# vvvvvw/Sentinel

Measured on AMD Instinct MI355X. Metric: decided entries/sec (whole node) at 1M resources; % of HBM roofline, higher is better.
Workload: dtype int64/f64

## Files before the change

sentinel_amd/csrc/decide.hip:

```cpp
#include <hip/hip_runtime.h>
#include <stdlib.h>
#include <stdint.h>

#include "authority.h"
#include "chain.h"
#include "aux.h"
#include "pmap.h"

using namespace sg;

#define WAVE 64
#define MAXR 16
#define JMAX_FLOW 4
#define JMAX_DEG 4
#define JMAX_RL 2

__device__ __forceinline__ uint32_t lane_id() { return __lane_id(); }
__device__ __forceinline__ uint64_t lanemask_lt() {
    uint32_t l = lane_id();
    return l == 0 ? 0ull : (~0ull >> (64 - l));
}

#define J8_MAX (1u << 23)
#define SEG_ITEMS 16
// ... 89 lines not shown
    if ((threadIdx.x & 63) == 63 && tot) base = atomicAdd(ctr, tot);
    base = __shfl(base, 63, 64);
    return base + x - k;
}
__global__ __launch_bounds__(256) void k_seg_bin(Seg* __restrict__ segs, const uint32_t* __restrict__ mp, uint64_t n,
                                                 const Prog* __restrict__ prog, const uint32_t* __restrict__ prio,
                                                 uint32_t lane_max, uint32_t j1_max,
                                                 uint32_t j4_max, uint32_t force_lane, uint32_t* __restrict__ blkcnt,
                                                 uint32_t nblk, uint32_t pq_ok, uint32_t pq_wide, uint32_t* __restrict__ aux,
                                                 uint32_t* __restrict__ ashort, uint64_t* __restrict__ along,
                                                 uint64_t* __restrict__ amulti, uint32_t* __restrict__ mixc,
                                                 uint32_t* __restrict__ mix, uint32_t mix_cap,
                                                 uint32_t* __restrict__ mixlen, uint32_t mix_wide, uint32_t head_min,
                                                 const uint16_t* __restrict__ hot_tab, uint32_t nhot,
                                                 const uint32_t* __restrict__ nhotseg, uint32_t* __restrict__ need_hot,
                                                 uint32_t* __restrict__ need_blk) {
    __shared__ uint32_t cnt[N_BINS];
    for (uint32_t b = threadIdx.x; b < N_BINS; b += blockDim.x) cnt[b] = 0;
    __syncthreads();
    const uint32_t m = *mp;
    const bool pq = pq_ok && !force_lane;
    const uint32_t s = blockIdx.x * blockDim.x + threadIdx.x;
    bool aux_short = false;
    uint32_t aux_np = 0;
    uint32_t mixk = 0;
    Seg sg;
    if (s < m) {
        sg = segs[s];
        const uint32_t end = (s + 1 < m) ? segs[s + 1].start : (uint32_t)n;
        sg.len = end - sg.start;
        const Prog p = prog[sg.res];
// ... 18 lines not shown
        else if (coop) bin = (sg.len > j4_max && (p.pflags & PF_J16))
                                 ? (((p.pflags & PF_FROZEN) && sg.len <= J8_MAX) ? BIN_J8 : BIN_J16)
                                 : sg.len > j1_max ? BIN_J4 : BIN_J1;
        else {
            int lb = 31 - __clz(sg.len | 1);
            if (lb > (int)LANE_BINS - 1) lb = LANE_BINS - 1;
            const bool lite = (p.n_param == 0 || ((p.xf & XF_PLITE) && !(pm & PM_ARGL))) && !p.multi && !lane_only &&
                              (p.pflags & PF_J16) && !(p.pflags & (PF_WARM | PF_SERIAL));
            bin = (lite ? BIN_LITE : (nr <= 4 && !inline_aux) ? BIN_LANE : BIN_LANE16) + (LANE_BINS - 1 - lb);
        }
        const bool auxp = aux && (pm & PM_AUX) && !(bin >= BIN_LANE16 && bin < BIN_LANE16 + LANE_BINS);
        if (auxp) {
            if (sg.len <= AUX_SHORT) aux_short = true;
            else aux_np = (sg.len + AUX_PIECE - 1) / AUX_PIECE;
        }
        const uint32_t rank = atomicAdd(&cnt[bin], 1u);
        sg.bin = bin | (auxp ? SEG_AUXP : 0u) | (rank << 8);
        segs[s] = sg;
        if (need_blk && (bin == BIN_J4 || bin == BIN_J8 || bin == BIN_J16) && sg.len) {
            if (s < *nhotseg) {
                const uint32_t hid = hot_tab[sg.res];
                if (hid < nhot) need_hot[hid] = 1u;
            } else {
                const uint32_t b0 = sg.start >> 10, b1 = (sg.start + sg.len - 1) >> 10;
                for (uint32_t wd = b0 >> 5; wd <= (b1 >> 5); ++wd) {
                    uint32_t m32 = 0xFFFFFFFFu;
                    if (wd == (b0 >> 5)) m32 &= 0xFFFFFFFFu << (b0 & 31);
                    if (wd == (b1 >> 5)) m32 &= 0xFFFFFFFFu >> (31 - (b1 & 31));
                    atomicOr(&need_blk[wd], m32);
                }
            }
        }
    }
    if (aux) {
        const uint32_t o = wave_alloc(aux + 0, aux_short ? 1u : 0u);
        if (aux_short) ashort[o] = s;
        const uint32_t q = wave_alloc(aux + 1, aux_np);
        const uint32_t j = wave_alloc(aux + 3, aux_np ? 1u : 0u);
        if (aux_np) along[j] = ((uint64_t)s << 32) | q;
        const uint32_t u = wave_alloc(aux + 2, aux_np > 1 ? 1u : 0u);
        if (aux_np > 1) amulti[u] = ((uint64_t)s << 32) | q;
    }
    if (mix) {
        const uint32_t a = wave_alloc(mixc + 0, mixk == 1 ? 1u : 0u);
        if (mixk == 1) mix[a] = s;
        const uint32_t b = wave_alloc(mixc + 1, mixk == 2 ? 1u : 0u);
        if (mixk == 2) mix[mix_cap + b] = s;
    }
    __syncthreads();
    for (uint32_t b = threadIdx.x; b < N_BINS; b += blockDim.x) blkcnt[(uint64_t)b * nblk + blockIdx.x] = cnt[b];
}
__global__ __launch_bounds__(256) void k_seg_order(Seg* __restrict__ segs, const uint32_t* __restrict__ mp,
                                                   const uint32_t* __restrict__ off, uint32_t nblk,
                                                   uint32_t* __restrict__ order) {
    const uint32_t s = blockIdx.x * blockDim.x + threadIdx.x;
    if (s >= *mp) return;
    const uint32_t v = segs[s].bin, bin = v & 0x7F;
    order[off[(uint64_t)bin * nblk + blockIdx.x] + (v >> 8)] = s;
    segs[s].bin = v & 0xFF;
}
__global__ void k_bin_offsets(const uint32_t* __restrict__ off, uint32_t nblk, const uint32_t* __restrict__ mp,
                              uint32_t* __restrict__ out) {
    const uint32_t b = threadIdx.x;
    if (b < N_BINS) out[b] = off[(uint64_t)b * nblk];
    if (b == N_BINS) out[b] = *mp;
}

__global__ __launch_bounds__(256) void k_scatter_rec(const SEv* __restrict__ rec_o, uint64_t n,
                                                     const uint32_t* __restrict__ pos_of, SEv* __restrict__ recs,
                                                     uint32_t* __restrict__ prev, uint32_t* __restrict__ nprev,
                                                     Link* __restrict__ link, uint32_t* __restrict__ bst, uint32_t epoch,
                                                     uint32_t* __restrict__ bflags) {
    const uint64_t i = (uint64_t)blockIdx.x * blockDim.x + threadIdx.x;
    if (i >= n) return;
// ... 1541 lines not shown
#define PROF_MARK(k)                                          \
    if (prof0) {                                              \
        unsigned long long _n = __builtin_amdgcn_s_memtime(); \
        tph[k] += _n - tmA;                                   \
        tmA = _n;                                             \
    }
#else
#define PROF_MARK(k)
#endif

    uint32_t tbase = 0;
    const uint32_t lp0 = tid * EP;
    SEv nxt[EP];
    JEv ev[EP];
    uint32_t gg[EP];
    const bool skip_on = SKIP && S.skip_ok && (pg.pflags & PF_FROZEN);
    auto in_span = [&](uint32_t rel) -> bool {
        if (!SKIP) return false;
        const uint32_t ns = sh.nsp;
        for (uint32_t i = 0; i < ns; ++i)
            if (rel >= sh.spn[i].x && rel < sh.spn[i].y) return true;
        return false;
    };
    auto decode = [&](const SEv& r, uint32_t pos) -> JEv {
        JEv x;
        const bool valid = pos < sg.len;
        x.dt = valid ? r.dt : 0;
        x.cz = (uint32_t)r.cnt | ((uint32_t)r.rt << 16);
        x.kf = valid ? ((uint32_t)r.kind | JK_VALID) : 0xFFu;
        if (valid && r.kind == SG_EV_ENTRY && (r.flags & RF_PBLK)) x.kf |= JK_PB;
        x.wi = 0;
// ... 1845 lines not shown
    hipLaunchKernelGGL(k_seg_emit, dim3(nt), dim3(256), 0, st, keys, n, pos, segs, lo, sbase);
    hipLaunchKernelGGL(k_add2, dim3(1), dim3(64), 0, st, nseg, sbase, ccount);
    return hipGetLastError();
}
hipError_t launch_block_sums(const SEv* recs, uint64_t n, uint32_t* bst, Link* link, uint32_t epoch, uint32_t* bflags,
                             const uint32_t* skeys, const uint32_t* lo, const uint32_t* need_blk, hipStream_t st) {
    hipLaunchKernelGGL(k_block_sums, dim3((uint32_t)((n + 1023) / 1024)), dim3(256), 0, st, recs, skeys, n, bst, link,
                       epoch, bflags, lo, need_blk);
    return hipGetLastError();
}
hipError_t launch_seg_bin(Seg* segs, const uint32_t* mp, uint32_t mb, uint64_t n, const Prog* prog, const uint32_t* prio,
                          uint32_t lane_max, uint32_t j1_max, uint32_t j4_max, uint32_t force_lane, uint32_t* blkcnt,
                          uint32_t pq_ok, uint32_t pq_wide, uint32_t* aux, uint32_t* ashort, uint64_t* along,
                          uint64_t* amulti, uint32_t* mixc, uint32_t* mix, uint32_t mix_cap, uint32_t* mixlen,
                          uint32_t mix_wide, uint32_t head_min, const uint16_t* hot_tab, uint32_t nhot,
                          const uint32_t* nhotseg, uint32_t* need_hot, uint32_t* need_blk, hipStream_t st) {
    const uint32_t nblk = (mb + 255) / 256;
    if (!nblk) return hipSuccess;
    hipLaunchKernelGGL(k_seg_bin, dim3(nblk), dim3(256), 0, st, segs, mp, n, prog, prio, lane_max, j1_max, j4_max, force_lane,
                       blkcnt, nblk, pq_ok, pq_wide, aux, ashort, along, amulti, mixc, mix, mix_cap, mixlen, mix_wide,
                       head_min, hot_tab, nhot, nhotseg, need_hot, need_blk);
    return hipGetLastError();
}
hipError_t launch_seg_order(Seg* segs, const uint32_t* mp, uint32_t mb, const uint32_t* off, uint32_t* order,
                            uint32_t* bin_off, hipStream_t st) {
    const uint32_t nblk = (mb + 255) / 256;
    if (nblk) hipLaunchKernelGGL(k_seg_order, dim3(nblk), dim3(256), 0, st, segs, mp, off, nblk, order);
    hipLaunchKernelGGL(k_bin_offsets, dim3(1), dim3(64), 0, st, off, nblk ? nblk : 1, mp, bin_off);
    return hipGetLastError();
}
hipError_t launch_gather(const SEv* rec_o, const uint32_t* vals, const uint32_t* skeys, uint64_t n,
                         const uint32_t* pos_of, SEv* recs, uint32_t* prev, uint32_t* nprev, Link* link, uint32_t* bst,
                         uint32_t epoch, uint32_t* bflags, hipStream_t st) {
    uint32_t nb = (uint32_t)((n + 255) / 256);
    hipError_t e = hipMemsetAsync(bst, 0, ((n + 1023) / 1024) * 4, st);
    if (e != hipSuccess) return e;
// ... 91 lines not shown
```

sentinel_amd/csrc/dev_types.h:

```cpp
#pragma once
#include <hip/hip_runtime.h>
#include <stdint.h>

#include "../../include/sentinel_gpu.h"

namespace sg {

struct AuthDesc;

struct Bkt {
    int64_t ws;
    int64_t pass;
    int64_t block;
    int64_t exc;
    int64_t succ;
    int64_t rt;
    int64_t occ;
    int64_t minrt;
};
static_assert(sizeof(Bkt) == 64, "Bkt must be 64 B");

#define NO_KEY 0xFFFFFFFFFFFFFFFFull

enum : uint32_t {
// ... 153 lines not shown
    int64_t snap_hi;
    uint64_t ring_mask;
    uint32_t dbg_flags;
    uint32_t heads;
};

struct Seg {
    uint32_t res;
    uint32_t start;
    uint32_t len;
    uint32_t bin;
};
#define SEG_AUXP 0x80u
#define SEG_PV 0x40u
#define SEG_PVT 0x100u

struct PvSeg {
    uint32_t ok;
    uint32_t n;
    uint32_t off;
    uint32_t mid;
    uint32_t rk;
    uint32_t ch0;
    uint32_t nch;
    uint32_t fbits;
    uint32_t freach;
    int32_t peak;
    uint32_t tm0;
    uint32_t sub;
};
// ... 210 lines not shown
```

sentinel_amd/csrc/engine.cpp:

```cpp
#include <hip/hip_runtime.h>

#include <algorithm>
#include <array>
#include <cmath>
#include <cstdint>
#include <cstdio>
#include <cstdlib>
#include <cstring>
#include <functional>
#include <map>
#include <set>
#include <string>
#include <unordered_map>
#include <vector>

#include "../../include/sentinel_gpu.h"
#include "authority.h"
#include "dev_types.h"
#include "pmap.h"

namespace sg {
hipError_t launch_rs_first(const sg_event* ev, uint64_t n, uint32_t max_res, uint64_t gbase, const uint8_t* ring,
                           uint64_t ring_mask, int32_t max_rt, SEv* rec_o, uint32_t* keys, uint32_t* vals,
                           uint32_t* ghist, uint32_t nblocks, uint32_t* bflags, int64_t* t0_out, uint32_t* prio,
// ... 6 lines not shown
                               uint32_t nblocks, hipStream_t st);
hipError_t launch_radix_scatter_n(const uint32_t* kin, const uint32_t* vin, uint64_t n, const uint32_t* ndev, int shift,
                                  const uint32_t* goff, uint32_t nblocks, uint32_t* kout, uint32_t* vout, hipStream_t st);
hipError_t launch_radix_scatter_x(const uint32_t* kin, const uint32_t* vin, uint64_t n, const uint32_t* ndev,
                                  const uint32_t* tcnt, const uint32_t* dbase, int shift, const uint32_t* goff,
                                  uint32_t nblocks, uint32_t* kout, uint32_t* vout, uint32_t* pos_of, hipStream_t st);
hipError_t launch_grp_first(const sg_event* ev, uint64_t n, uint32_t max_res, uint64_t gbase, uint64_t ring_mask,
                            uint32_t* bflags, int64_t* t0_out, uint32_t* prio, uint64_t* key_ring, const uint32_t* comp,
                            const sg_event_ext* ext, const sg_arg* args, uint64_t n_args, uint32_t max_ctx,
                            const AuthDesc* auth, const uint32_t* auth_ids,
                            const uint16_t* hot_tab, uint32_t nhot, uint32_t nblocks, uint32_t* words,
                            uint32_t* hot_hist, uint32_t* ckeys, uint32_t* cvals, uint32_t* ccnt, uint32_t* chist,
                            hipStream_t st);
hipError_t launch_hot_scan(uint32_t* C, uint32_t nblocks, uint32_t nhot, uint32_t* part, uint32_t* hb, uint32_t* total,
                           hipStream_t st);
hipError_t launch_grp_records(const sg_event* ev, uint64_t n, uint64_t gbase, uint64_t ring_mask, int32_t max_rt,
                              const uint32_t* words, const uint32_t* P, uint32_t nhot, uint32_t nblocks,
                              const uint32_t* hb, SEv* recs, uint32_t* svals, uint32_t* prev,
                              uint32_t* nprev, uint32_t* bst, uint32_t* bflags, const sg_event_ext* ext,
                              const sg_arg* args, uint32_t max_ctx, Link* link, uint32_t epoch,
                              const uint32_t* need_hot, const uint32_t* need_blk, hipStream_t st);
hipError_t launch_hot_segs(const uint32_t* hb, uint32_t nhot, const uint32_t* hot_list, Seg* segs, uint32_t* out,
                           hipStream_t st);
hipError_t launch_hot_build(const Seg* segs, const uint32_t* mp, uint32_t mb, uint32_t min_len, uint32_t max_res, uint16_t* hot_tab,
                            uint32_t* hot_list, uint32_t nhot_old, uint32_t* hot_n, hipStream_t st);
hipError_t launch_cold_n(uint64_t n, const uint32_t* hot_total, uint32_t* out, hipStream_t st);
hipError_t launch_cold_small(const uint32_t* kin, const uint32_t* vin, const uint32_t* cnt, const uint32_t* dbase,
                             uint32_t* kout, uint32_t* vout, uint32_t* words, hipStream_t st);
uint32_t hot_max();
hipError_t launch_seg_cold(const uint32_t* keys, uint64_t n, const uint32_t* lo, const uint32_t* sbase, uint32_t* flag,
// ... 7 lines not shown
uint32_t radix_tile();
hipError_t launch_scan(const uint32_t*, uint32_t*, uint64_t, uint32_t*, uint32_t*, hipStream_t);
hipError_t launch_snapshot(Bkt*, NodeInfo*, uint32_t, int64_t, int32_t, uint32_t*, uint32_t*, uint32_t*, uint32_t*,
                           sg_metric_node*, uint64_t, hipStream_t);
hipError_t launch_init_state(Bkt* sec, Bkt* minb, NodeInfo* info, int64_t* borrow, uint32_t nres, hipStream_t st);
hipError_t launch_set_flags(NodeInfo* info, const uint64_t* upd, uint32_t n, hipStream_t st);
hipError_t launch_region_copy(const uint64_t* src, uint64_t* dst, const uint64_t* tri, uint32_t n, hipStream_t st);
hipError_t launch_seg(const uint32_t* keys, uint64_t n, uint32_t* flag, uint32_t* pos, Seg* segs, hipStream_t st,
                      hipError_t (*scan)(const uint32_t*, uint32_t*, uint64_t, uint32_t*, uint32_t*, hipStream_t),
                      uint32_t* part, uint32_t* nseg);
hipError_t launch_seg_bin(Seg* segs, const uint32_t* mp, uint32_t mb, uint64_t n, const Prog* prog, const uint32_t* prio,
                          uint32_t lane_max, uint32_t j1_max, uint32_t j4_max, uint32_t force_lane, uint32_t* blkcnt,
                          uint32_t pq_ok, uint32_t pq_wide, uint32_t* aux, uint32_t* ashort, uint64_t* along,
                          uint64_t* amulti, uint32_t* mixc, uint32_t* mix, uint32_t mix_cap, uint32_t* mixlen,
                          uint32_t mix_wide, uint32_t head_min, const uint16_t* hot_tab, uint32_t nhot,
                          const uint32_t* nhotseg, uint32_t* need_hot, uint32_t* need_blk, hipStream_t st);
hipError_t launch_aux(const SEv* recs, const Seg* segs, const uint32_t* aux, const uint32_t* ashort,
                      const uint64_t* along, uint64_t* apiece, const uint64_t* amulti, const DevState& S, const DevCfg& cfg,
                      int64_t t0, const uint32_t* dec, AuxAcc* pool, uint32_t pool_cap, uint32_t* pool_n, uint64_t* meta,
                      uint32_t* bflags, hipStream_t st);
hipError_t launch_aux_cold(const SEv* recs, const Seg* segs, const uint32_t* aux, const uint32_t* ashort, const DevState& S,
                           const DevCfg& cfg, int64_t t0, const uint32_t* dec, uint32_t* bflags, hipStream_t st);
hipError_t launch_pq(int wide, const SEv* recs, const sg_event* ev, const uint32_t* vals, const Seg* segs,
                     const uint32_t* order, uint32_t m, const DevState& S, const DevCfg& cfg, int64_t t0, uint32_t* dec,
                     uint32_t* bflags, hipStream_t st);
hipError_t launch_pm_grow(const Seg* segs, const uint32_t* mp, uint32_t mb, const DevState& S, unsigned long long* pool_next,
                          uint64_t pool_nb, uint32_t* bflags, uint4* mv, uint32_t* nmv, uint32_t mcap, uint32_t epoch,
                          uint32_t nm, PBucket* b2, PData* d2, uint32_t* sz, uint32_t* off, uint32_t* part,
                          hipError_t (*scan)(const uint32_t*, uint32_t*, uint64_t, uint32_t*, uint32_t*, hipStream_t),
                          hipStream_t st);
hipError_t launch_pm_compact(PMap* pm, uint32_t n, const PBucket* ob, const PData* od, PBucket* nbk, PData* nd,
// ... 442 lines not shown
    uint32_t* d_ppre = nullptr;
    uint32_t* d_tmid = nullptr;
    uint8_t* d_ring = nullptr;
    uint32_t rules_cap = 0, hot_cap = 0;

    struct BatchSlot {
        sg_event* d_ev = nullptr;
        uint32_t* d_out = nullptr;
        uint32_t *d_k0 = nullptr, *d_v0 = nullptr, *d_k1 = nullptr, *d_v1 = nullptr;
        uint32_t *d_hist = nullptr, *d_part = nullptr, *d_flag = nullptr, *d_pos = nullptr, *d_order = nullptr;
        uint32_t *d_posof = nullptr, *d_dec = nullptr, *d_blkcnt = nullptr, *d_prev = nullptr;
        SEv *d_recs = nullptr, *d_rec_o = nullptr;
        uint32_t* d_ccnt = nullptr;
        bool radix = false;
        uint32_t nhot = 0;
        Seg* d_segs = nullptr;
        uint64_t* d_cand = nullptr;
        uint32_t* d_bsmall = nullptr;
        sg_event_ext* d_ext = nullptr;
        sg_arg* d_args = nullptr;
        uint64_t ext_cap = 0, args_cap = 0;
        uint32_t* d_ashort = nullptr;
        uint64_t *d_apiece = nullptr, *d_amulti = nullptr, *d_along = nullptr;
        uint64_t aux_cap_n = 0;
        uint32_t* d_mix = nullptr;
        uint64_t mix_cap = 0;
        Link* d_link = nullptr;
        uint32_t *d_bst = nullptr, *d_pend = nullptr;
        Span* d_spans = nullptr;
        hipEvent_t ev[5] = {nullptr, nullptr, nullptr, nullptr, nullptr};
        bool pending = false;
    } slot[2];
    int cur = 0;
    int last = -1;
    hipStream_t gstream = nullptr;
    std::vector<std::array<double, 4>> tlog;
    std::string fatal;
    uint32_t* d_prio = nullptr;
    uint16_t* d_hot_tab = nullptr;
    uint32_t* d_hot_list = nullptr;
    uint32_t nhot = 0;
    uint32_t* d_hot_part = nullptr;
    uint32_t* d_hot_hb = nullptr;
    uint32_t* d_need = nullptr;
    uint64_t need_words = 0;
    bool radix_group = false;
    uint64_t radix_below = 1u << 18;
    uint32_t tok_light = 8192;
    uint32_t tok_wide = 1024;
    bool tiny_on = true;
    AuxNode* d_auxtab = nullptr;
    uint32_t* d_auxcnt = nullptr;
    uint64_t aux_mask = 0;
    AuxAcc* d_auxpool = nullptr;
    uint64_t* d_auxmeta = nullptr;
    uint32_t auxpool_cap = 0;
    uint64_t auxmeta_cap = 0;
    std::unordered_map<std::string, uint32_t> origin_ids, context_ids;
    std::unordered_map<std::string, int> rule_names;
    AuthTable auth;
// ... 147 lines not shown
        HIPCHK(hipMalloc(&B.d_flag, c * 4));
        HIPCHK(hipMalloc(&B.d_pos, c * 4));
        HIPCHK(hipMalloc(&B.d_order, c * 4));
        HIPCHK(hipMalloc(&B.d_segs, c * sizeof(Seg)));
        HIPCHK(hipMalloc(&B.d_cand, c * 8));
        HIPCHK(hipMalloc(&B.d_posof, c * 4));
        HIPCHK(hipMalloc(&B.d_dec, c * 4));
        HIPCHK(hipMalloc(&B.d_recs, c * sizeof(SEv)));
        const uint64_t co = (e->radix_group || c >= (1ull << 30)) ? c : std::min<uint64_t>(c, e->radix_below);
        if (co) HIPCHK(hipMalloc(&B.d_rec_o, co * sizeof(SEv)));
        HIPCHK(hipMalloc(&B.d_ccnt, 3 * (nblocks + 64) * 4));
    }
    dfree(e->d_hot_part);
    dfree(e->d_hot_hb);
    dfree(e->d_need);
    e->need_words = hot_max() + c / 32768 + 2;
    HIPCHK(hipMalloc(&e->d_need, e->need_words * 4));
    HIPCHK(hipMalloc(&e->d_hot_part, (nblocks / 16 + 2) * hot_max() * 4));
    HIPCHK(hipMalloc(&e->d_hot_hb, 2 * hot_max() * 4));
    for (auto& B : e->slot) {
        HIPCHK(hipMalloc(&B.d_blkcnt, ((c + 255) / 256 + 1) * N_BINS * 4));
        HIPCHK(hipMalloc(&B.d_prev, c * 4));
        HIPCHK(hipMalloc(&B.d_bsmall, 256 * 4));
        HIPCHK(hipMemset(B.d_bsmall, 0, 256 * 4));
        HIPCHK(hipMalloc(&B.d_link, c * sizeof(Link)));
        HIPCHK(hipMemset(B.d_link, 0, c * sizeof(Link)));
        HIPCHK(hipMalloc(&B.d_bst, ((c + 1023) / 1024 + 1) * 4));
        HIPCHK(hipMalloc(&B.d_pend, c * 4));
        HIPCHK(hipMalloc(&B.d_spans, (c / SPAN_CHUNK + 65536) * sizeof(Span)));
    }
    e->span_cap = (uint32_t)(c / SPAN_CHUNK + 65536);
    e->cap_n = c;
// ... 8 lines not shown
    HIPCHK(hipEventSynchronize(B.ev[4]));
    float g = 0, d = 0, p = 0;
    (void)hipEventElapsedTime(&g, B.ev[0], B.ev[1]);
    (void)hipEventElapsedTime(&d, B.ev[2], B.ev[3]);
    (void)hipEventElapsedTime(&p, B.ev[3], B.ev[4]);
    (void)hipGetLastError();
    e->last_ms[0] = g; e->last_ms[1] = d; e->last_ms[2] = p; e->last_ms[3] = (double)g + d + p;
    e->tlog.push_back({(double)g, (double)d, (double)p, (double)g + d + p});
    if (e->tlog.size() > 4096) e->tlog.erase(e->tlog.begin(), e->tlog.begin() + 2048);
    uint32_t bflags = 0;
    HIPCHK(hipMemcpyAsync(&bflags, B.d_bsmall, 4, hipMemcpyDeviceToHost, e->gstream));
    uint32_t nspan = 0;
    HIPCHK(hipMemcpyAsync(&nspan, B.d_bsmall + 120, 4, hipMemcpyDeviceToHost, e->gstream));
    HIPCHK(hipStreamSynchronize(e->gstream));
    e->spans_total += nspan;
    if (bflags & BF_BAD_REF)
        return fail(SG_EINVAL, "an EXIT/TRACE references an event that is not an earlier ENTRY of the same resource");
    if (bflags & BF_BACKWARD)
        return fail(SG_EINVAL, "event timestamps must be non-decreasing across batches (SURVEY Q3)");
    if (bflags & BF_AUX_FULL) return fail(SG_ECAPACITY, "origin/context node pool full (raise aux_node_capacity)");
    if (bflags & BF_LITE_STALE)
        return fail(SG_ESTATE, "internal error (SG_LITE_CHECK): k_lite stored a minute bucket without a load that was not stale");
    if (bflags & BF_PQ_INVARIANT)
        e->fatal = "internal error: a k_pq tile's presorted key subset did not match its accesses";
    else if (bflags & BF_POOL_FULL)
        e->fatal = "the hot-parameter map pool is used up (raise param_table_log2)";
    else if (bflags & BF_PTAB_FULL)
        e->fatal = "a hot-parameter map table could not place a key (its map holds a ghost entry)";
    if (bflags & (BF_PQ_INVARIANT | BF_PTAB_FULL | BF_POOL_FULL)) return fail(SG_ECAPACITY, e->fatal + " -- engine unusable");
    return SG_OK;
// ... 475 lines not shown

extern "C" int sgx_timing_log(sg_engine* e, double* out, int cap) {
    if (!e || !out) return 0;
    (void)drain(e);
    int k = 0;
    for (; k < cap && k < (int)e->tlog.size(); ++k)
        for (int j = 0; j < 4; ++j) out[4 * k + j] = e->tlog[k][j];
    e->tlog.clear();
    return k;
}
extern "C" unsigned long long sgx_spans_total(sg_engine* e) {
    if (!e) return 0;
    (void)drain(e);
    return e->spans_total;
}
extern "C" int sgx_debug_reset(sg_engine* e) {
    if (!e || !e->d_dbg) return 0;
    (void)drain(e);
    unsigned long long z[64] = {0};
    z[20] = ~0ull;
    return hipMemcpy(e->d_dbg, z, sizeof(z), hipMemcpyHostToDevice) == hipSuccess ? 1 : 0;
}
extern "C" int sgx_debug_counters(sg_engine* e, unsigned long long* out, int cap) {
    if (!e || !e->d_dbg || !out) return 0;
    int k = cap < 64 ? cap : 64;
    if (hipDeviceSynchronize() != hipSuccess) return 0;
    if (hipMemcpy(out, e->d_dbg, (size_t)k * 8, hipMemcpyDeviceToHost) != hipSuccess) return 0;
    return k;
}

// ... 61 lines not shown

int sg_engine_destroy(sg_engine* e) {
    if (!e) return SG_OK;
    (void)hipSetDevice(e->device);
    if (e->stream) (void)hipStreamSynchronize(e->stream);
    if (e->gstream) (void)hipStreamSynchronize(e->gstream);
    dfree(e->d_sec); dfree(e->d_minb); dfree(e->d_info); dfree(e->d_prog); dfree(e->d_rules); dfree(e->d_rstate);
    dfree(e->d_hot); dfree(e->d_pmap); dfree(e->d_pbkt); dfree(e->d_pdat); dfree(e->d_pbm); dfree(e->d_ppre); dfree(e->d_tmid); dfree(e->d_ring); dfree(e->d_small); dfree(e->d_sink);
    dfree(e->d_pool_next); dfree(e->d_pmoves); dfree(e->d_pbkt2); dfree(e->d_pdat2); dfree(e->d_pcwork);
    if (e->h_pool_next) (void)hipHostFree(e->h_pool_next);
    free_pv(e);
    dfree(e->d_pvseg); dfree(e->d_pvtseg); dfree(e->d_pvtot); dfree(e->d_pvrest);
    if (e->gstream) (void)hipStreamSynchronize(e->gstream);
    for (auto& B : e->slot) free_slot(B);
    dfree(e->d_auth); dfree(e->d_auth_ids);
    dfree(e->d_prio); dfree(e->d_hot_tab); dfree(e->d_hot_list); dfree(e->d_hot_part); dfree(e->d_hot_hb); dfree(e->d_need); dfree(e->d_comp); dfree(e->d_auxtab); dfree(e->d_auxpool); dfree(e->d_auxcnt); dfree(e->d_auxmeta);
    dfree(e->d_pflow); dfree(e->d_phot); dfree(e->d_pftab); dfree(e->d_pvtab); dfree(e->d_preq); dfree(e->d_pvals);
    dfree(e->d_cflow); dfree(e->d_cbkt); dfree(e->d_ctab); dfree(e->d_nslim); dfree(e->d_nslimit); dfree(e->d_nsb); dfree(e->d_borrow); dfree(e->d_keyring);
    dfree(e->d_treq); dfree(e->d_tres); dfree(e->d_tfidx); dfree(e->d_tbounds);
    dfree(e->d_snap_cnt); dfree(e->d_snap_off); dfree(e->d_snap_out); dfree(e->d_dbg);
    for (auto& B : e->slot)
        for (auto& v : B.ev) if (v) (void)hipEventDestroy(v);
    if (e->gstream) (void)hipStreamDestroy(e->gstream);
    for (auto& v : e->join) if (v) (void)hipEventDestroy(v);
    if (e->fork) (void)hipEventDestroy(e->fork);
    if (e->fork0) (void)hipEventDestroy(e->fork0);
    if (e->grown) (void)hipEventDestroy(e->grown);
    for (auto& s : e->bin_stream) if (s) (void)hipStreamDestroy(s);
    if (e->stream) (void)hipStreamDestroy(e->stream);
    delete e;
    return SG_OK;
// ... 841 lines not shown
    int64_t* d_t0 = reinterpret_cast<int64_t*>(e->d_bsmall + 4);
    uint32_t *kin = e->d_k1, *vin = e->d_v1, *kout = e->d_k0, *vout = e->d_v0;
    if (++e->epoch == 0) e->epoch = 1;
    B.radix = e->radix_group || n >= (1ull << 30) || n < e->radix_below;
    const bool force_lane = !e->cfg.switch_on || (e->dbg_flags & 2);
    const uint32_t mb = (uint32_t)std::min<uint64_t>(n, R);
    const uint32_t nblk = (mb + 255) / 256;
    uint32_t lane_max = e->lane_max, j1_max = e->j1_max, j4_max = e->j4_max;
    if (!e->bins_pinned && n < SHARD_BATCH) {
        lane_max = std::min<uint32_t>(lane_max, 128);
        j1_max = std::min<uint32_t>(j1_max, 1024);
        j4_max = std::min<uint32_t>(j4_max, 4096);
    }
    j1_max = std::min<uint32_t>(j1_max, 64u * 65000u);
    j4_max = std::min<uint32_t>(j4_max, 256u * 65000u);
    auto bins = [&](uint32_t* need_hot, uint32_t* need_blk) -> int {
        if (ext) {
            if (int arc = ensure_aux(e, B, n)) return arc;
        }
        if (e->has_mix) {
            if (int mrc = ensure_mix(B, mb)) return mrc;
        }
        HIPCHK(launch_seg_bin(e->d_segs, e->d_bsmall + 1, mb, n, e->d_prog, e->d_prio, lane_max, j1_max, j4_max,
                              force_lane ? 1 : 0, e->d_blkcnt, e->pq_on ? 1u : 0u, e->pq_wide, ext ? e->d_bsmall + 130 : nullptr,
                              B.d_ashort, B.d_along, B.d_amulti, e->d_bsmall + 6, e->has_mix ? B.d_mix : nullptr,
                              (uint32_t)B.mix_cap, e->d_bsmall + 72, (e->pv_on || e->pvt_on) ? 0u : e->pq_wide,
                              (e->dbg_flags & HEAD_OFF) ? 0u : e->head_min, e->d_hot_tab, e->nhot, e->d_bsmall + 80, need_hot,
                              need_blk, gs));
        HIPCHK(launch_scan(e->d_blkcnt, e->d_blkcnt, (uint64_t)nblk * N_BINS, e->d_part, nullptr, gs));
        HIPCHK(launch_seg_order(e->d_segs, e->d_bsmall + 1, mb, e->d_blkcnt, e->d_order, e->d_bsmall + 8, gs));
        return SG_OK;
    };
    if (B.radix) {
        HIPCHK(launch_rs_first(dev_ev, n, R, e->gbase, e->d_ring, ring_mask, e->cfg.statistic_max_rt, e->d_rec_o,
                               e->d_k1, e->d_v1, e->d_hist, nblocks, e->d_bsmall + 0, d_t0, e->d_prio, e->d_keyring,
                               e->d_comp, dev_ext, dev_args, n_args, SG_MAX_CONTEXTS, dev_auth(e), dev_auth_ids(e), gs));
        for (int p = 0; p < passes; ++p) {
            if (p > 0) HIPCHK(launch_radix_hist(kin, n, p * db, e->d_hist, nblocks, gs));
            HIPCHK(launch_scan(e->d_hist, e->d_hist, (uint64_t)nblocks << db, e->d_part, nullptr, gs));
            HIPCHK(launch_radix_scatter(kin, vin, n, p * db, e->d_hist, nblocks, kout, vout,
                                        p == passes - 1 ? e->d_posof : nullptr, gs));
            std::swap(kin, kout);
            std::swap(vin, vout);
        }
        HIPCHK(launch_seg(kin, n, e->d_flag, e->d_pos, e->d_segs, gs, launch_scan, e->d_part, e->d_bsmall + 1));
        HIPCHK(launch_gather(e->d_rec_o, vin, kin, n, e->d_posof, e->d_recs, e->d_prev, e->d_bsmall + 3, e->d_link,
                             e->d_bst, e->epoch, e->d_bsmall + 0, gs));
        if (int brc = bins(nullptr, nullptr)) return brc;
    } else {
        const uint32_t nhot = e->nhot;
        B.nhot = nhot;
        uint32_t* words = e->d_flag;
        uint32_t* hot_off = e->d_pos;
        uint32_t* ccnt = B.d_ccnt;
        HIPCHK(launch_grp_first(dev_ev, n, R, e->gbase, ring_mask, e->d_bsmall + 0, d_t0, e->d_prio, e->d_keyring,
                                e->d_comp, dev_ext, dev_args, n_args, SG_MAX_CONTEXTS, dev_auth(e), dev_auth_ids(e),
                                e->d_hot_tab, nhot, nblocks,
                                words, hot_off, e->d_k1, e->d_v1, ccnt, e->d_hist, gs));
        HIPCHK(launch_hot_scan(hot_off, nblocks, nhot, e->d_hot_part, e->d_hot_hb, e->d_bsmall + 77, gs));
        HIPCHK(launch_cold_n(n, e->d_bsmall + 77, e->d_bsmall + 78, gs));
        if (nblocks == 1) {
            HIPCHK(launch_cold_small(kin, vin, ccnt, e->d_bsmall + 77, kout, vout, words, gs));
            std::swap(kin, kout);
// ... 2 lines not shown
        for (int p = 0; p < passes && nblocks > 1; ++p) {
            if (p > 0) HIPCHK(launch_radix_hist_n(kin, n, e->d_bsmall + 78, p * db, e->d_hist, nblocks, gs));
            HIPCHK(launch_scan(e->d_hist, e->d_hist, (uint64_t)nblocks << db, e->d_part, nullptr, gs));
            const bool last = p == passes - 1;
            HIPCHK(launch_radix_scatter_x(kin, vin, n, p ? e->d_bsmall + 78 : nullptr, p ? nullptr : ccnt,
                                          last ? e->d_bsmall + 77 : nullptr, p * db, e->d_hist, nblocks, kout, vout,
                                          last ? words : nullptr, gs));
            std::swap(kin, kout);
            std::swap(vin, vout);
        }
        HIPCHK(launch_hot_segs(e->d_hot_hb, nhot, e->d_hot_list, e->d_segs, e->d_bsmall + 80, gs));
        const uint64_t sc = nblocks + 64;
        HIPCHK(launch_seg_cold(kin, n, e->d_bsmall + 77, e->d_bsmall + 80, ccnt + sc, ccnt + 2 * sc, e->d_segs, gs,
                               launch_scan, e->d_part, e->d_bsmall + 82, e->d_bsmall + 1));
        HIPCHK(hipMemsetAsync(e->d_bst, 0, ((n + 1023) / 1024) * 4, gs));
        uint32_t *need_hot = nullptr, *need_blk = nullptr;
        if (!(e->dbg_flags & TABLES_ALL)) {
            need_hot = e->d_need;
            need_blk = e->d_need + hot_max();
            HIPCHK(hipMemsetAsync(e->d_need, 0, e->need_words * 4, gs));
        }
        if (int brc = bins(need_hot, need_blk)) return brc;
        HIPCHK(launch_grp_records(dev_ev, n, e->gbase, ring_mask, e->cfg.statistic_max_rt, words, hot_off, nhot, nblocks,
                                  e->d_hot_hb, e->d_recs, vin, e->d_prev, e->d_bsmall + 3, e->d_bst,
                                  e->d_bsmall + 0, dev_ext, dev_args, SG_MAX_CONTEXTS, e->d_link, e->epoch, need_hot,
                                  need_blk, gs));
        HIPCHK(launch_block_sums(e->d_recs, n, e->d_bst, e->d_link, e->epoch, e->d_bsmall + 0, kin, e->d_bsmall + 77,
                                 need_blk, gs));
    }
    const uint32_t hot_min = (uint32_t)std::max<uint64_t>(64, n / 8192);
    if (!B.radix)
        HIPCHK(launch_hot_build(e->d_segs, e->d_bsmall + 1, mb, hot_min, R, e->d_hot_tab, e->d_hot_list, e->nhot,
                                e->d_bsmall + 76, gs));
    uint32_t head[77];
    static_assert(8 + N_BINS + 1 <= 72, "head layout");
    HIPCHK(hipMemcpyAsync(head, e->d_bsmall, sizeof(head), hipMemcpyDeviceToHost, gs));
    HIPCHK(hipEventRecord(B.ev[1], gs));
    HIPCHK(hipStreamSynchronize(gs));
    if (!B.radix) e->nhot = std::min<uint32_t>(head[76], hot_max());
    const uint32_t m = head[1];
    const uint32_t nprev = head[3];
    int64_t t0 = 0;
    std::memcpy(&t0, head + 4, 8);
    uint32_t bflags = head[0];
    if (bflags & BF_BAD_RES) return fail(SG_EINVAL, "event res_id >= max_resources");
    if (bflags & BF_BAD_REF)
        return fail(SG_EINVAL, "an EXIT/TRACE references an event that is not an earlier ENTRY of the same resource");
    if (bflags & BF_TSPAN) return fail(SG_EINVAL, "a batch must span less than 2^31 ms");
    if (bflags & BF_BACKWARD) return fail(SG_EINVAL, "event timestamps must be non-decreasing (SURVEY Q3)");
    if (bflags & BF_BAD_ARGS)
        return fail(SG_EINVAL, "an sg_event_ext names args outside the table (or more than SG_MAX_ARGS, or a bad kind)");
    const uint32_t* off = head + 8;
    uint32_t bin_n[N_BINS];
    for (int b = 0; b < N_BINS; ++b) bin_n[b] = off[b + 1] - off[b];
// ... 24 lines not shown
    S.tmid = e->d_tmid;
    S.ring = e->d_ring;
    S.sink = e->d_sink;
    S.borrow = e->d_borrow;
    S.prio = e->d_prio;
    S.key_ring = e->d_keyring;
    S.gbase = e->gbase;
    S.link = e->d_link;
    S.bst = e->d_bst;
    S.pend = e->d_pend;
    S.spans = e->d_spans;
    S.nspan = e->d_bsmall + 120;
    S.span_cap = e->span_cap;
    S.epoch = e->epoch;
    S.skip_ok = !(bflags & (BF_MULTI_LINK | BF_ZERO_CNT)) && !(e->dbg_flags & 4) ? 1u : 0u;
    S.skip_min = (!e->skip_pinned && n < SHARD_BATCH) ? std::min<uint32_t>(e->skip_min, 8192) : e->skip_min;
    S.ext = dev_ext;
    S.args = dev_args;
    S.aux_tab = e->d_auxtab;
    S.aux_count = e->d_auxcnt;
    S.aux_cap = e->cfg.aux_node_capacity;
    S.aux_mask = e->aux_mask;
    S.max_ctx = SG_MAX_CONTEXTS;
    S.auth = dev_auth(e);
    S.auth_ids = dev_auth_ids(e);
    HIPCHK(hipStreamWaitEvent(st, B.ev[1], 0));
    const uint32_t n_mix = e->has_mix ? head[6] : 0u, n_mixw = e->has_mix ? head[7] : 0u;
    const bool serial_bins = (e->dbg_flags & 8) != 0;
    const bool pre_split = (n_mix || n_mixw) && !serial_bins;
    hipStream_t ps = pre_split ? e->bin_stream[1] : st;
    const uint32_t grant_all = (e->cfg.switch_on && e->cfg.max_slot_chain_size <= 0) ? 1u : 0u;
// ... 807 lines not shown
```

sentinel_amd/csrc/kernels.hip:

```cpp
#include <hip/hip_runtime.h>
#include <stdint.h>
#include <stdlib.h>

#include "../../include/sentinel_gpu.h"
#include "authority.h"
#include "dev_types.h"

using namespace sg;

#define WAVE 64

#define RS_THREADS 256
#ifndef RS_ITEMS
#define RS_ITEMS 16
#endif
#define RS_TILE (RS_THREADS * RS_ITEMS)
#define RS_BINS 256

template <int DB>
__device__ __forceinline__ void hist_add(uint32_t* h, uint32_t d, bool valid) {
    uint64_t peers = __ballot(valid);
#pragma unroll
    for (int b = 0; b < DB; ++b) {
        const uint64_t bb = __ballot((d >> b) & 1);
// ... 319 lines not shown
    if (h == 0) *out = all;
}
__global__ __launch_bounds__(256) void k_hot_scan_c(uint32_t* __restrict__ C, uint32_t nblocks, uint32_t nhot,
                                                    const uint32_t* __restrict__ part, const uint32_t* __restrict__ hb) {
    const uint32_t c = blockIdx.x, t0 = c * HS_TC, t1 = min(nblocks, t0 + HS_TC);
    for (uint32_t h = threadIdx.x; h < nhot; h += 256) {
        uint32_t run = hb[h] + part[(uint64_t)c * nhot + h];
        for (uint32_t t = t0; t < t1; ++t) {
            const uint32_t v = C[(uint64_t)t * nhot + h];
            C[(uint64_t)t * nhot + h] = run;
            run += v;
        }
    }
}

__device__ __forceinline__ uint32_t grp_pos(uint64_t j, uint32_t wd, const uint32_t* __restrict__ P, uint32_t nhot) {
    if (wd & W_HOT) return P[(j / RS_TILE) * nhot + ((wd >> 12) & (HOT_MAX - 1))] + (wd & 0xFFFu);
    return wd & W_POS;
}

#define GR_THREADS 256
#define GR_EVENTS (RS_TILE / 4)
#define GR_ITEMS (GR_EVENTS / GR_THREADS)
__global__ __launch_bounds__(GR_THREADS) void k_grp_records(const sg_event* __restrict__ ev, uint64_t n,
                                                            uint64_t gbase, uint64_t ring_mask, int32_t max_rt,
                                                            const uint32_t* __restrict__ words,
                                                            const uint32_t* __restrict__ P, uint32_t nhot,
                                                            uint32_t nblocks, const uint32_t* __restrict__ hb,
                                                            SEv* __restrict__ recs,
                                                            uint32_t* __restrict__ svals, uint32_t* __restrict__ prev,
// ... 648 lines not shown
                            hipStream_t st) {
    hipLaunchKernelGGL(k_grp_first<8>, dim3(nblocks), dim3(RS_THREADS), 0, st, ev, n, max_res, gbase, ring_mask, bflags,
                       t0_out, prio, key_ring, comp, ext, args, n_args, max_ctx, auth, auth_ids, hot_tab, nhot, nblocks, words,
                       hot_hist, ckeys, cvals, ccnt, chist);
    return hipGetLastError();
}
hipError_t launch_hot_scan(uint32_t* C, uint32_t nblocks, uint32_t nhot, uint32_t* part, uint32_t* hb, uint32_t* total,
                           hipStream_t st) {
    if (!nhot) return hipMemsetAsync(total, 0, 4, st);
    const uint32_t nch = (nblocks + HS_TC - 1) / HS_TC;
    hipLaunchKernelGGL(k_hot_scan_a, dim3(nch), dim3(256), 0, st, C, nblocks, nhot, part);
    hipLaunchKernelGGL(k_hot_scan_b, dim3(1), dim3(HOT_MAX), 0, st, part, nch, nhot, hb, total);
    hipLaunchKernelGGL(k_hot_scan_c, dim3(nch), dim3(256), 0, st, C, nblocks, nhot, part, hb);
    return hipGetLastError();
}
hipError_t launch_grp_records(const sg_event* ev, uint64_t n, uint64_t gbase, uint64_t ring_mask, int32_t max_rt,
                              const uint32_t* words, const uint32_t* P, uint32_t nhot, uint32_t nblocks,
                              const uint32_t* hb, SEv* recs, uint32_t* svals, uint32_t* prev,
                              uint32_t* nprev, uint32_t* bst, uint32_t* bflags, const sg_event_ext* ext,
                              const sg_arg* args, uint32_t max_ctx, Link* link, uint32_t epoch,
                              const uint32_t* need_hot, const uint32_t* need_blk, hipStream_t st) {
    hipLaunchKernelGGL(k_grp_records, dim3(nblocks * 4), dim3(GR_THREADS), 0, st, ev, n, gbase, ring_mask, max_rt, words, P,
                       nhot, nblocks, hb, recs, svals, prev, nprev, bst, bflags, ext, args, max_ctx, link, epoch, need_hot,
                       need_blk);
    return hipGetLastError();
}
hipError_t launch_hot_segs(const uint32_t* hb, uint32_t nhot, const uint32_t* hot_list, Seg* segs, uint32_t* out,
                           hipStream_t st) {
    hipLaunchKernelGGL(k_hot_segs, dim3(1), dim3(HOT_MAX), 0, st, hb, nhot, hot_list, segs, out);
    return hipGetLastError();
// ... 134 lines not shown
```

sentinel_amd/engine.py:

```python
from __future__ import annotations

import ctypes as C
import os

import numpy as np

from . import _abi as A

_HERE = os.path.dirname(os.path.abspath(__file__))
LIB_PATH = os.environ.get("SG_LIB_PATH") or os.path.join(_HERE, "libsentinel_gpu.so")
_lib = None

EXPORTS = (
    "sg_config_default", "sg_engine_create", "sg_engine_destroy", "sg_register_resources", "sg_resource_id",
    "sg_load_flow_rules", "sg_load_degrade_rules", "sg_load_param_rules", "sg_param_key", "sg_submit",
    "sg_submit_async", "sg_sync", "sg_snapshot_metrics", "sg_cluster_set_connected_count",
    "sg_cluster_request_tokens", "sg_cluster_request_param_tokens", "sg_read_node", "sg_last_error", "sg_last_timings",
    "sg_submit_ex", "sg_submit_ex_async", "sg_intern_origin", "sg_intern_context", "sg_param_thread_count",
    "sg_cluster_namespace", "sg_cluster_assign_flows", "sg_cluster_set_namespace_connected",
    "sg_cluster_namespace_qps", "sg_load_authority_rules",
)


class SentinelError(RuntimeError):
# ... 171 lines not shown

    def timing_log(self, cap: int = 4096) -> np.ndarray:
        buf = (C.c_double * (4 * cap))()
        fn = lib().sgx_timing_log
        fn.restype = C.c_int
        fn.argtypes = [C.c_void_p, C.c_void_p, C.c_int]
        k = fn(self.h, buf, cap)
        return np.frombuffer(buf, dtype=np.float64, count=4 * k).reshape(k, 4).copy()

    def spans_total(self) -> int:
        fn = lib().sgx_spans_total
        fn.restype = C.c_ulonglong
        fn.argtypes = [C.c_void_p]
        return int(fn(self.h))

    def read_aux_node(self, res: int, kind: int, node_id: int):
        fn = lib().sgx_read_aux_node
        fn.restype = C.c_int
        fn.argtypes = [C.c_void_p, C.c_uint32, C.c_uint32, C.c_uint32, C.c_void_p]
        out = np.zeros(21, dtype=np.int64)
        rc = fn(self.h, res, kind, node_id, out.ctypes.data)
        if rc < 0:
            raise SentinelError(A.SG_EDEVICE, "sgx_read_aux_node failed")
        if rc == 0:
            return None
        return {"second": out[:16].reshape(2, 8), "thread": int(out[16]), "mhist": out[17:21].reshape(2, 2)}

    def pv_last(self) -> dict:
        fn = lib().sgx_pv_last
        fn.restype = C.c_int
# ... 99 lines not shown
```

Baseline: 4.277 billion.

## Only build skip tables for hot segments whose per-bucket span exceeds threshold

Adds a pre-pass that finds time-bucket edges (500-unit buckets) over tile heads and computes, per hot resource, the largest per-bucket count. Segment binning then marks need_hot/need_blk only when that count (or the segment length for cold ones) exceeds a skip threshold scaled by the bin's cooperation width, and it tags such segments with SEG_TABS. The decide kernel enables the skip path only for tagged segments. This avoids building and consulting skip tables for segments too small to benefit, at the cost of two extra small kernels, one of them single-block, plus a wider rank shift in the segment bin field.

```diff
diff --git a/sentinel_amd/csrc/decide.hip b/sentinel_amd/csrc/decide.hip
--- a/sentinel_amd/csrc/decide.hip
+++ b/sentinel_amd/csrc/decide.hip
@@ -127,7 +127,8 @@
                                                  uint32_t* __restrict__ mixlen, uint32_t mix_wide, uint32_t head_min,
                                                  const uint16_t* __restrict__ hot_tab, uint32_t nhot,
                                                  const uint32_t* __restrict__ nhotseg, uint32_t* __restrict__ need_hot,
-                                                 uint32_t* __restrict__ need_blk) {
+                                                 uint32_t* __restrict__ need_blk, const uint32_t* __restrict__ bmax,
+                                                 uint32_t skip_min, uint32_t* __restrict__ nmark) {
     __shared__ uint32_t cnt[N_BINS];
     for (uint32_t b = threadIdx.x; b < N_BINS; b += blockDim.x) cnt[b] = 0;
     __syncthreads();
@@ -176,14 +177,18 @@
             if (sg.len <= AUX_SHORT) aux_short = true;
             else aux_np = (sg.len + AUX_PIECE - 1) / AUX_PIECE;
         }
-        const uint32_t rank = atomicAdd(&cnt[bin], 1u);
-        sg.bin = bin | (auxp ? SEG_AUXP : 0u) | (rank << 8);
-        segs[s] = sg;
+        bool tabs = !need_blk;
         if (need_blk && (bin == BIN_J4 || bin == BIN_J8 || bin == BIN_J16) && sg.len) {
+            const uint32_t nw = bin == BIN_J4 ? 4u : bin == BIN_J8 ? 8u : 16u;
+            const uint32_t thr = skip_min * nw / 16 > 0 ? skip_min * nw / 16 : 1u;
             if (s < *nhotseg) {
                 const uint32_t hid = hot_tab[sg.res];
-                if (hid < nhot) need_hot[hid] = 1u;
-            } else {
+                if (hid < nhot && bmax[hid] > thr) {
+                    need_hot[hid] = 1u;
+                    atomicAdd(nmark, 1u);
+                    tabs = true;
+                }
+            } else if (sg.len > thr) {
                 const uint32_t b0 = sg.start >> 10, b1 = (sg.start + sg.len - 1) >> 10;
                 for (uint32_t wd = b0 >> 5; wd <= (b1 >> 5); ++wd) {
                     uint32_t m32 = 0xFFFFFFFFu;
@@ -191,8 +196,12 @@
                     if (wd == (b1 >> 5)) m32 &= 0xFFFFFFFFu >> (31 - (b1 & 31));
                     atomicOr(&need_blk[wd], m32);
                 }
-            }
-        }
+                tabs = true;
+            }
+        }
+        const uint32_t rank = atomicAdd(&cnt[bin], 1u);
+        sg.bin = bin | (auxp ? SEG_AUXP : 0u) | (tabs ? SEG_TABS : 0u) | (rank << SEG_RANK_SHIFT);
+        segs[s] = sg;
     }
     if (aux) {
         const uint32_t o = wave_alloc(aux + 0, aux_short ? 1u : 0u);
@@ -217,9 +226,9 @@
                                                    uint32_t* __restrict__ order) {
     const uint32_t s = blockIdx.x * blockDim.x + threadIdx.x;
     if (s >= *mp) return;
-    const uint32_t v = segs[s].bin, bin = v & 0x7F;
-    order[off[(uint64_t)bin * nblk + blockIdx.x] + (v >> 8)] = s;
-    segs[s].bin = v & 0xFF;
+    const uint32_t v = segs[s].bin, bin = v & 0x3F;
+    order[off[(uint64_t)bin * nblk + blockIdx.x] + (v >> SEG_RANK_SHIFT)] = s;
+    segs[s].bin = v & ((1u << SEG_RANK_SHIFT) - 1);
 }
 __global__ void k_bin_offsets(const uint32_t* __restrict__ off, uint32_t nblk, const uint32_t* __restrict__ mp,
                               uint32_t* __restrict__ out) {
@@ -1791,7 +1800,7 @@
     SEv nxt[EP];
     JEv ev[EP];
     uint32_t gg[EP];
-    const bool skip_on = SKIP && S.skip_ok && (pg.pflags & PF_FROZEN);
+    const bool skip_on = SKIP && S.skip_ok && (pg.pflags & PF_FROZEN) && (sg.bin & SEG_TABS);
     auto in_span = [&](uint32_t rel) -> bool {
         if (!SKIP) return false;
         const uint32_t ns = sh.nsp;
@@ -3667,12 +3676,13 @@
                           uint32_t pq_ok, uint32_t pq_wide, uint32_t* aux, uint32_t* ashort, uint64_t* along,
                           uint64_t* amulti, uint32_t* mixc, uint32_t* mix, uint32_t mix_cap, uint32_t* mixlen,
                           uint32_t mix_wide, uint32_t head_min, const uint16_t* hot_tab, uint32_t nhot,
-                          const uint32_t* nhotseg, uint32_t* need_hot, uint32_t* need_blk, hipStream_t st) {
+                          const uint32_t* nhotseg, uint32_t* need_hot, uint32_t* need_blk, const uint32_t* bmax,
+                          uint32_t skip_min, uint32_t* nmark, hipStream_t st) {
     const uint32_t nblk = (mb + 255) / 256;
     if (!nblk) return hipSuccess;
     hipLaunchKernelGGL(k_seg_bin, dim3(nblk), dim3(256), 0, st, segs, mp, n, prog, prio, lane_max, j1_max, j4_max, force_lane,
                        blkcnt, nblk, pq_ok, pq_wide, aux, ashort, along, amulti, mixc, mix, mix_cap, mixlen, mix_wide,
-                       head_min, hot_tab, nhot, nhotseg, need_hot, need_blk);
+                       head_min, hot_tab, nhot, nhotseg, need_hot, need_blk, bmax, skip_min, nmark);
     return hipGetLastError();
 }
 hipError_t launch_seg_order(Seg* segs, const uint32_t* mp, uint32_t mb, const uint32_t* off, uint32_t* order,
diff --git a/sentinel_amd/csrc/dev_types.h b/sentinel_amd/csrc/dev_types.h
--- a/sentinel_amd/csrc/dev_types.h
+++ b/sentinel_amd/csrc/dev_types.h
@@ -191,6 +191,8 @@
 #define SEG_AUXP 0x80u
 #define SEG_PV 0x40u
 #define SEG_PVT 0x100u
+#define SEG_TABS 0x200u
+#define SEG_RANK_SHIFT 10
 
 struct PvSeg {
     uint32_t ok;
diff --git a/sentinel_amd/csrc/engine.cpp b/sentinel_amd/csrc/engine.cpp
--- a/sentinel_amd/csrc/engine.cpp
+++ b/sentinel_amd/csrc/engine.cpp
@@ -44,6 +44,8 @@
                             hipStream_t st);
 hipError_t launch_hot_scan(uint32_t* C, uint32_t nblocks, uint32_t nhot, uint32_t* part, uint32_t* hb, uint32_t* total,
                            hipStream_t st);
+hipError_t launch_hot_bmax(const sg_event* ev, uint32_t nblocks, const uint32_t* P, uint32_t nhot, const uint32_t* hb,
+                           uint32_t* edges, uint32_t* bmax, hipStream_t st);
 hipError_t launch_grp_records(const sg_event* ev, uint64_t n, uint64_t gbase, uint64_t ring_mask, int32_t max_rt,
                               const uint32_t* words, const uint32_t* P, uint32_t nhot, uint32_t nblocks,
                               const uint32_t* hb, SEv* recs, uint32_t* svals, uint32_t* prev,
@@ -81,7 +83,8 @@
                           uint32_t pq_ok, uint32_t pq_wide, uint32_t* aux, uint32_t* ashort, uint64_t* along,
                           uint64_t* amulti, uint32_t* mixc, uint32_t* mix, uint32_t mix_cap, uint32_t* mixlen,
                           uint32_t mix_wide, uint32_t head_min, const uint16_t* hot_tab, uint32_t nhot,
-                          const uint32_t* nhotseg, uint32_t* need_hot, uint32_t* need_blk, hipStream_t st);
+                          const uint32_t* nhotseg, uint32_t* need_hot, uint32_t* need_blk, const uint32_t* bmax,
+                          uint32_t skip_min, uint32_t* nmark, hipStream_t st);
 hipError_t launch_aux(const SEv* recs, const Seg* segs, const uint32_t* aux, const uint32_t* ashort,
                       const uint64_t* along, uint64_t* apiece, const uint64_t* amulti, const DevState& S, const DevCfg& cfg,
                       int64_t t0, const uint32_t* dec, AuxAcc* pool, uint32_t pool_cap, uint32_t* pool_n, uint64_t* meta,
@@ -554,6 +557,7 @@
         uint32_t* d_ccnt = nullptr;
         bool radix = false;
         uint32_t nhot = 0;
+        uint32_t hot_marked = 0;
         Seg* d_segs = nullptr;
         uint64_t* d_cand = nullptr;
         uint32_t* d_bsmall = nullptr;
@@ -584,6 +588,8 @@
     uint32_t* d_hot_hb = nullptr;
     uint32_t* d_need = nullptr;
     uint64_t need_words = 0;
+    uint32_t* d_edges = nullptr;
+    uint32_t hot_marked_last = 0;
     bool radix_group = false;
     uint64_t radix_below = 1u << 18;
     uint32_t tok_light = 8192;
@@ -761,8 +767,10 @@
     dfree(e->d_hot_part);
     dfree(e->d_hot_hb);
     dfree(e->d_need);
-    e->need_words = hot_max() + c / 32768 + 2;
+    dfree(e->d_edges);
+    e->need_words = hot_max() + c / 32768 + 2 + hot_max();
     HIPCHK(hipMalloc(&e->d_need, e->need_words * 4));
+    HIPCHK(hipMalloc(&e->d_edges, (nblocks + 2) * 4));
     HIPCHK(hipMalloc(&e->d_hot_part, (nblocks / 16 + 2) * hot_max() * 4));
     HIPCHK(hipMalloc(&e->d_hot_hb, 2 * hot_max() * 4));
     for (auto& B : e->slot) {
@@ -801,6 +809,7 @@
     HIPCHK(hipMemcpyAsync(&nspan, B.d_bsmall + 120, 4, hipMemcpyDeviceToHost, e->gstream));
     HIPCHK(hipStreamSynchronize(e->gstream));
     e->spans_total += nspan;
+    e->hot_marked_last = B.hot_marked;
     if (bflags & BF_BAD_REF)
         return fail(SG_EINVAL, "an EXIT/TRACE references an event that is not an earlier ENTRY of the same resource");
     if (bflags & BF_BACKWARD)
@@ -1306,6 +1315,11 @@
     (void)drain(e);
     return e->spans_total;
 }
+extern "C" unsigned int sgx_hot_marked(sg_engine* e) {
+    if (!e) return 0;
+    (void)drain(e);
+    return e->hot_marked_last;
+}
 extern "C" int sgx_debug_reset(sg_engine* e) {
     if (!e || !e->d_dbg) return 0;
     (void)drain(e);
@@ -1397,7 +1411,7 @@
     if (e->gstream) (void)hipStreamSynchronize(e->gstream);
     for (auto& B : e->slot) free_slot(B);
     dfree(e->d_auth); dfree(e->d_auth_ids);
-    dfree(e->d_prio); dfree(e->d_hot_tab); dfree(e->d_hot_list); dfree(e->d_hot_part); dfree(e->d_hot_hb); dfree(e->d_need); dfree(e->d_comp); dfree(e->d_auxtab); dfree(e->d_auxpool); dfree(e->d_auxcnt); dfree(e->d_auxmeta);
+    dfree(e->d_prio); dfree(e->d_hot_tab); dfree(e->d_hot_list); dfree(e->d_hot_part); dfree(e->d_hot_hb); dfree(e->d_need); dfree(e->d_edges); dfree(e->d_comp); dfree(e->d_auxtab); dfree(e->d_auxpool); dfree(e->d_auxcnt); dfree(e->d_auxmeta);
     dfree(e->d_pflow); dfree(e->d_phot); dfree(e->d_pftab); dfree(e->d_pvtab); dfree(e->d_preq); dfree(e->d_pvals);
     dfree(e->d_cflow); dfree(e->d_cbkt); dfree(e->d_ctab); dfree(e->d_nslim); dfree(e->d_nslimit); dfree(e->d_nsb); dfree(e->d_borrow); dfree(e->d_keyring);
     dfree(e->d_treq); dfree(e->d_tres); dfree(e->d_tfidx); dfree(e->d_tbounds);
@@ -2269,7 +2283,8 @@
     }
     j1_max = std::min<uint32_t>(j1_max, 64u * 65000u);
     j4_max = std::min<uint32_t>(j4_max, 256u * 65000u);
-    auto bins = [&](uint32_t* need_hot, uint32_t* need_blk) -> int {
+    const uint32_t skip_min = (!e->skip_pinned && n < SHARD_BATCH) ? std::min<uint32_t>(e->skip_min, 8192) : e->skip_min;
+    auto bins = [&](uint32_t* need_hot, uint32_t* need_blk, const uint32_t* bmax) -> int {
         if (ext) {
             if (int arc = ensure_aux(e, B, n)) return arc;
         }
@@ -2281,7 +2296,7 @@
                               B.d_ashort, B.d_along, B.d_amulti, e->d_bsmall + 6, e->has_mix ? B.d_mix : nullptr,
                               (uint32_t)B.mix_cap, e->d_bsmall + 72, (e->pv_on || e->pvt_on) ? 0u : e->pq_wide,
                               (e->dbg_flags & HEAD_OFF) ? 0u : e->head_min, e->d_hot_tab, e->nhot, e->d_bsmall + 80, need_hot,
-                              need_blk, gs));
+                              need_blk, bmax, skip_min, e->d_bsmall + 73, gs));
         HIPCHK(launch_scan(e->d_blkcnt, e->d_blkcnt, (uint64_t)nblk * N_BINS, e->d_part, nullptr, gs));
         HIPCHK(launch_seg_order(e->d_segs, e->d_bsmall + 1, mb, e->d_blkcnt, e->d_order, e->d_bsmall + 8, gs));
         return SG_OK;
@@ -2301,7 +2316,7 @@
         HIPCHK(launch_seg(kin, n, e->d_flag, e->d_pos, e->d_segs, gs, launch_scan, e->d_part, e->d_bsmall + 1));
         HIPCHK(launch_gather(e->d_rec_o, vin, kin, n, e->d_posof, e->d_recs, e->d_prev, e->d_bsmall + 3, e->d_link,
                              e->d_bst, e->epoch, e->d_bsmall + 0, gs));
-        if (int brc = bins(nullptr, nullptr)) return brc;
+        if (int brc = bins(nullptr, nullptr, nullptr)) return brc;
     } else {
         const uint32_t nhot = e->nhot;
         B.nhot = nhot;
@@ -2334,13 +2349,15 @@
         HIPCHK(launch_seg_cold(kin, n, e->d_bsmall + 77, e->d_bsmall + 80, ccnt + sc, ccnt + 2 * sc, e->d_segs, gs,
                                launch_scan, e->d_part, e->d_bsmall + 82, e->d_bsmall + 1));
         HIPCHK(hipMemsetAsync(e->d_bst, 0, ((n + 1023) / 1024) * 4, gs));
-        uint32_t *need_hot = nullptr, *need_blk = nullptr;
+        uint32_t *need_hot = nullptr, *need_blk = nullptr, *bmax = nullptr;
         if (!(e->dbg_flags & TABLES_ALL)) {
             need_hot = e->d_need;
             need_blk = e->d_need + hot_max();
+            bmax = e->d_need + e->need_words - hot_max();
             HIPCHK(hipMemsetAsync(e->d_need, 0, e->need_words * 4, gs));
-        }
-        if (int brc = bins(need_hot, need_blk)) return brc;
+            HIPCHK(launch_hot_bmax(dev_ev, nblocks, hot_off, nhot, e->d_hot_hb, e->d_edges, bmax, gs));
+        }
+        if (int brc = bins(need_hot, need_blk, bmax)) return brc;
         HIPCHK(launch_grp_records(dev_ev, n, e->gbase, ring_mask, e->cfg.statistic_max_rt, words, hot_off, nhot, nblocks,
                                   e->d_hot_hb, e->d_recs, vin, e->d_prev, e->d_bsmall + 3, e->d_bst,
                                   e->d_bsmall + 0, dev_ext, dev_args, SG_MAX_CONTEXTS, e->d_link, e->epoch, need_hot,
@@ -2358,6 +2375,7 @@
     HIPCHK(hipEventRecord(B.ev[1], gs));
     HIPCHK(hipStreamSynchronize(gs));
     if (!B.radix) e->nhot = std::min<uint32_t>(head[76], hot_max());
+    B.hot_marked = head[73];
     const uint32_t m = head[1];
     const uint32_t nprev = head[3];
     int64_t t0 = 0;
@@ -2412,7 +2430,7 @@
     S.span_cap = e->span_cap;
     S.epoch = e->epoch;
     S.skip_ok = !(bflags & (BF_MULTI_LINK | BF_ZERO_CNT)) && !(e->dbg_flags & 4) ? 1u : 0u;
-    S.skip_min = (!e->skip_pinned && n < SHARD_BATCH) ? std::min<uint32_t>(e->skip_min, 8192) : e->skip_min;
+    S.skip_min = skip_min;
     S.ext = dev_ext;
     S.args = dev_args;
     S.aux_tab = e->d_auxtab;
diff --git a/sentinel_amd/csrc/kernels.hip b/sentinel_amd/csrc/kernels.hip
--- a/sentinel_amd/csrc/kernels.hip
+++ b/sentinel_amd/csrc/kernels.hip
@@ -357,6 +357,64 @@
     }
 }
 
+#define BE_THREADS 1024
+#define BE_ITEMS 8
+__global__ __launch_bounds__(BE_THREADS) void k_bkt_edges(const sg_event* __restrict__ ev, uint32_t nblocks,
+                                                          uint32_t* __restrict__ edges) {
+    __shared__ uint32_t ws[BE_THREADS / 64];
+    const uint32_t t = threadIdx.x, l = t & 63, wv = t >> 6;
+    uint32_t run = 0;
+    for (uint32_t c0 = 0; c0 < nblocks; c0 += BE_THREADS * BE_ITEMS) {
+        const uint32_t t0 = c0 + t * BE_ITEMS;
+        int64_t ts[BE_ITEMS + 1];
+#pragma unroll
+        for (int k = 0; k <= BE_ITEMS; ++k) {
+            uint32_t tl = (t0 + k) ? t0 + k - 1 : 0u;
+            if (tl >= nblocks) tl = nblocks - 1;
+            ts[k] = ev[(uint64_t)tl * RS_TILE].ts;
+        }
+        uint32_t f = 0;
+#pragma unroll
+        for (int k = 0; k < BE_ITEMS; ++k)
+            if (t0 + k < nblocks && (t0 + k == 0 || ts[k + 1] / 500 != ts[k] / 500)) f |= 1u << k;
+        const uint32_t c = (uint32_t)__popc(f);
+        uint32_t x = c;
+#pragma unroll
+        for (int o = 1; o < 64; o <<= 1) {
+            const uint32_t y = __shfl_up(x, o, 64);
+            if ((int)l >= o) x += y;
+        }
+        if (l == 63) ws[wv] = x;
+        __syncthreads();
+        uint32_t pre = 0, all = 0;
+        for (uint32_t k = 0; k < BE_THREADS / 64; ++k) { if (k < wv) pre += ws[k]; all += ws[k]; }
+        uint32_t o = 1 + run + pre + x - c;
+#pragma unroll
+        for (int k = 0; k < BE_ITEMS; ++k)
+            if ((f >> k) & 1u) edges[o++] = t0 + k;
+        run += all;
+        __syncthreads();
+    }
+    if (t == 0) edges[0] = run;
+}
+#define BM_EDGES 32u
+__global__ __launch_bounds__(256) void k_hot_bmax(const uint32_t* __restrict__ P, uint32_t nblocks, uint32_t nhot,
+                                                  const uint32_t* __restrict__ hb, const uint32_t* __restrict__ edges,
+                                                  uint32_t* __restrict__ bmax) {
+    const uint32_t ne = edges[0], j0 = blockIdx.y * BM_EDGES, j1 = min(ne, j0 + BM_EDGES);
+    const uint32_t h = blockIdx.x * 256 + threadIdx.x;
+    if (j0 >= ne || h >= nhot) return;
+    const uint32_t end = hb[h] + hb[HOT_MAX + h];
+    uint32_t m = 0;
+    for (uint32_t j = j0; j < j1; ++j) {
+        const uint32_t a = edges[1 + j], b = j + 1 < ne ? edges[2 + j] : nblocks;
+        const uint32_t lo = P[(uint64_t)(a ? a - 1 : 0u) * nhot + h];
+        const uint32_t hi = b < nblocks ? P[(uint64_t)b * nhot + h] : end;
+        m = max(m, hi - lo);
+    }
+    if (m) atomicMax(&bmax[h], m);
+}
+
 __device__ __forceinline__ uint32_t grp_pos(uint64_t j, uint32_t wd, const uint32_t* __restrict__ P, uint32_t nhot) {
     if (wd & W_HOT) return P[(j / RS_TILE) * nhot + ((wd >> 12) & (HOT_MAX - 1))] + (wd & 0xFFFu);
     return wd & W_POS;
@@ -1035,6 +1093,14 @@
     hipLaunchKernelGGL(k_hot_scan_c, dim3(nch), dim3(256), 0, st, C, nblocks, nhot, part, hb);
     return hipGetLastError();
 }
+hipError_t launch_hot_bmax(const sg_event* ev, uint32_t nblocks, const uint32_t* P, uint32_t nhot, const uint32_t* hb,
+                           uint32_t* edges, uint32_t* bmax, hipStream_t st) {
+    if (!nhot || !nblocks) return hipSuccess;
+    hipLaunchKernelGGL(k_bkt_edges, dim3(1), dim3(BE_THREADS), 0, st, ev, nblocks, edges);
+    hipLaunchKernelGGL(k_hot_bmax, dim3((nhot + 255) / 256, (nblocks + BM_EDGES - 1) / BM_EDGES), dim3(256), 0, st, P,
+                       nblocks, nhot, hb, edges, bmax);
+    return hipGetLastError();
+}
 hipError_t launch_grp_records(const sg_event* ev, uint64_t n, uint64_t gbase, uint64_t ring_mask, int32_t max_rt,
                               const uint32_t* words, const uint32_t* P, uint32_t nhot, uint32_t nblocks,
                               const uint32_t* hb, SEv* recs, uint32_t* svals, uint32_t* prev,
diff --git a/sentinel_amd/engine.py b/sentinel_amd/engine.py
--- a/sentinel_amd/engine.py
+++ b/sentinel_amd/engine.py
@@ -209,6 +209,12 @@
         fn.argtypes = [C.c_void_p]
         return int(fn(self.h))
 
+    def hot_marked(self) -> int:
+        fn = lib().sgx_hot_marked
+        fn.restype = C.c_uint
+        fn.argtypes = [C.c_void_p]
+        return int(fn(self.h))
+
     def read_aux_node(self, res: int, kind: int, node_id: int):
         fn = lib().sgx_read_aux_node
         fn.restype = C.c_int
```

Result: faster. 4.497 billion (median of 6 runs) (+5.1%).
